# SvenGronauer/distributedTensorFlow

Hardware: AMD Instinct MI355X
Metric: images/sec (whole node) ResNet-50 synthetic ImageNet at 1/2/4/8 MI355X (higher is better)
Workload: dtype bf16; 1 GPU; model=resnet50, global_batch=1984, per_gpu_batch=1984, image_size=224, parallelism=dp1, impl=dtf, optimizer=momentum0.9+wd1e-4, lr 0.1*B/256 warmup500+cosine, backend=auto, native_ext=distributedtensorflow_amd/_lib/_dtf_hip.cpython-310-x86_64-linux-gnu.so

## Files before the change

csrc/kernels/gemm.hip:

```cpp
#include <algorithm>
#include <stdexcept>
#include <string>

#include "launch.h"

namespace {

constexpr int kGT = 512;
constexpr uint32_t kGOOB = 0xFFFFFFF0u;

struct GemmArgs {
  const bf16_t* A; const bf16_t* B; bf16_t* C;
  const float* bias;
  const bf16_t* Cin;
  int M, N, K, lda, ldb, ldc;
  int relu;
  float* stats;
  const bf16_t* acc_src;
  const uint8_t* acc_mask;
  int H, W, Cc, P, Q, sh, sw, ntaps;
  int tdh[9], tdw[9];
  int Ho, Wo, osh, osw, oh0, ow0;
  int nt;
  int dbg;
  const bf16_t* gelu_a;
  const float* gelu_b;
  float* colsum;
  bf16_t* gelu_out;
  int ncu;
  int group_m;
  int stagger_mode, stagger;
};

template <int BK>
DTF_DEV int gswz(int row, int ch) {
  constexpr int CPR = BK / 8, RPB = 16 / CPR;
  return ch ^ ((row / RPB) % CPR);
}

template <int BM, int BN, int BK, int NS, int NW = 8>
struct GCfg {
  static constexpr int NT = NW * 64;
  static constexpr int WN = NW == 8 ? BN / 64 : 2, WM = NW / WN;
  static constexpr int WTM = BM / WM, WTN = BN / WN;
  static constexpr int FM = WTM / 16, FN = WTN / 16;
  static constexpr int CPR = BK / 8;
  static constexpr int RPI = 64 / CPR;
  static constexpr int DA = BM / RPI / NW, DB = BN / RPI / NW;
  static constexpr int SA = BM * BK, STAGE = (BM + BN) * BK;
  static constexpr int LDC = BN + 8;
  static constexpr size_t EPI = (size_t)BM * LDC * 2 + (size_t)WM * 2 * BN * 4;
  static constexpr size_t LDS = (size_t)NS * STAGE * 2 > EPI ? (size_t)NS * STAGE * 2 : EPI;
};

template <int BM, int BN, int BK, int NS, int SCHED = 0, int NW = 8, int PP_PRIO = 1,
          int CONV = 0, int OCC = 1>
__global__ void __launch_bounds__(NW * 64, OCC == 2 ? NW * 2 / 4 : 1)
gemm_nt_kernel(const GemmArgs g) {
  using Cf = GCfg<BM, BN, BK, NS, NW>;
  extern __shared__ __attribute__((aligned(16))) bf16_t lds[];
  const int tid = threadIdx.x, lane = tid & 63;
  const int wave = __builtin_amdgcn_readfirstlane(tid >> 6);
  const int wm = wave / Cf::WN, wn = wave % Cf::WN;
  (void)kGT;

  const int tiles_n = (g.N + BN - 1) / BN;
  const int tiles_m = (g.M + BM - 1) / BM;
  const int bid = xcd_remap(blockIdx.x, tiles_n * tiles_m);
  int tm, tn;
  if (g.group_m > 0) {
    const int per = g.group_m * tiles_n, grp = bid / per, first = grp * g.group_m;
    const int gm = min(g.group_m, tiles_m - first), r = bid - grp * per;
    tm = first + r % gm;
    tn = r / gm;
  } else {
    tm = bid / tiles_n;
    tn = bid % tiles_n;
  }
  const int m0 = tm * BM, n0 = tn * BN;
  const int nk = (g.K + BK - 1) / BK;
  if constexpr (OCC == 2) {
    const int b = blockIdx.x;
    const bool late = b < 2 * g.ncu &&
        (g.stagger_mode == 1 ? b >= g.ncu
         : g.stagger_mode == 2 ? ((b >> 3) & 1) != 0
         : g.stagger_mode == 3 ? (b & 1) != 0 : false);
    if (late)
      for (int i = 0; i < g.stagger; ++i) __builtin_amdgcn_s_sleep(127);
  }

  const int rows_a = min(BM, g.M - m0), rows_b = min(BN, g.N - n0);
  const int PQc = CONV ? g.P * g.Q : 1;
  const int n_lo = CONV ? m0 / PQc : 0;
  const long img = CONV ? (long)g.H * g.W * g.Cc : 0;
  const i32x4_t ra =
      CONV ? rsrc_quad(g.A + n_lo * img,
                       (uint32_t)(((m0 + rows_a - 1) / PQc - n_lo + 1) * img * 2))
           : rsrc_quad(g.A + (long)m0 * g.lda, (uint32_t)((long)(rows_a - 1) * g.lda + g.K) * 2u);
  const i32x4_t rb = rsrc_quad(g.B + (long)n0 * g.ldb, (uint32_t)((long)(rows_b - 1) * g.ldb + g.K) * 2u);
  const uint32_t lds0 = lds_addr(lds);

  const int lrow = lane / Cf::CPR, slot = lane % Cf::CPR;
  uint32_t a_off[Cf::DA], b_off[Cf::DB];
  int a_ch[Cf::DA], b_ch[Cf::DB];
// ... 762 lines not shown
        float v[4];
        bf16_t h[4];
#pragma unroll
        for (int r = 0; r < 4; ++r) {
          v[r] = acc[i][j][r] + b4[r];
          if (g.relu) v[r] = fmaxf(v[r], 0.f);
          h[r] = f2bf(v[r]);
          if (do_stats && ok) {
            const float qv = bf2f(h[r]);
            s1[r] += qv;
            s2[r] += qv * qv;
          }
        }
        const long eoff = rowoff[i] + ncol;
        if (ok && (g.Cin || g.acc_mask)) {
          const bf16_t* src = g.Cin ? g.Cin + cbase + eoff : g.acc_src + cbase + eoff;
          const uint2 sv = *reinterpret_cast<const uint2*>(src);
          const uint32_t bits = g.Cin ? 0xFu
                                      : (g.acc_mask[(cbase + eoff) >> 3] >> ((cbase + eoff) & 7)) & 0xFu;
          const float s[4] = {__builtin_bit_cast(float, sv.x << 16),
                              __builtin_bit_cast(float, sv.x & 0xffff0000u),
                              __builtin_bit_cast(float, sv.y << 16),
                              __builtin_bit_cast(float, sv.y & 0xffff0000u)};
#pragma unroll
          for (int r = 0; r < 4; ++r) h[r] = f2bf(bf2f(h[r]) + ((bits >> r) & 1u ? s[r] : 0.f));
        }
        typedef uint32_t u32x2_t __attribute__((ext_vector_type(2)));
        const u32x2_t w = {(uint32_t)h[0] | ((uint32_t)h[1] << 16),
                           (uint32_t)h[2] | ((uint32_t)h[3] << 16)};
        const int so = ok ? (int)(eoff * 2) : (int)kGOOB;
        if (nt_store) __builtin_amdgcn_raw_buffer_store_b64(w, rc, so, 0, 2);
        else __builtin_amdgcn_raw_buffer_store_b64(w, rc, so, 0, 0);
      }
      if (do_stats) {
#pragma unroll
        for (int r = 0; r < 4; ++r) {
#pragma unroll
          for (int o = 1; o < 16; o <<= 1) {
            s1[r] += __shfl_xor(s1[r], o, 64);
            s2[r] += __shfl_xor(s2[r], o, 64);
          }
        }
        if (frow == 0) {
          const int col = wn * 64 + j * 16 + fq * 4;
#pragma unroll
          for (int r = 0; r < 4; ++r) {
            red[(wm * 2 + 0) * BN + col + r] = s1[r];
            red[(wm * 2 + 1) * BN + col + r] = s2[r];
          }
        }
      }
    }
    if (do_stats) {
      asm volatile("s_waitcnt lgkmcnt(0)" ::: "memory");
      raw_barrier();
      if (tid < BN && cur.n0 + tid < g.N) {
        float a = 0.f, b = 0.f;
#pragma unroll
        for (int k = 0; k < Cf::WM; ++k) { a += red[(k * 2 + 0) * BN + tid]; b += red[(k * 2 + 1) * BN + tid]; }
        const int tm = cur.m0 / BM;
        g.stats[((long)tm * 2 + 0) * g.N + cur.n0 + tid] = a;
        g.stats[((long)tm * 2 + 1) * g.N + cur.n0 + tid] = b;
      }
      asm volatile("s_waitcnt lgkmcnt(0)" ::: "memory");
      raw_barrier();
    }
    if (!nxt_valid) break;
#pragma unroll
    for (int i = 0; i < Cf::FM; ++i)
#pragma unroll
      for (int j = 0; j < Cf::FN; ++j) acc[i][j] = (f32x4_t){0.f, 0.f, 0.f, 0.f};
    gstep0 += nk;
    cur = tile_of(seq + 1);
    nxt_valid = tile_of(seq + 2).valid;
    ra = desc_a(cur);
    rb = desc_b(cur);
    cache();
    first = false;
    static_assert(NSTORE == 32, "the counted waits below assume 32 stores per lane per tile");
  }
  DTF_WAIT_VM(0);
}

template <int CONV, int EPI>
__global__ void __launch_bounds__(512, 1)
gemm_pp2_kernel(const GemmArgs g) {
  using Cf = GCfg<256, 256, 64, 2, 8>;
  constexpr int BM = 256, BN = 256, BK = 64;
  constexpr int NSTORE = Cf::FM * Cf::FN;
  extern __shared__ __attribute__((aligned(16))) bf16_t lds[];
  const int tid = threadIdx.x, lane = tid & 63;
  const int wave = __builtin_amdgcn_readfirstlane(tid >> 6);
  const int wm = wave / Cf::WN, wn = wave % Cf::WN;
  const int tiles_n = (g.N + BN - 1) / BN, tiles_m = (g.M + BM - 1) / BM;
  const int ntiles = tiles_n * tiles_m;
  const int nk = g.K / BK;
  const uint32_t lds0 = lds_addr(lds);
  const int lrow = lane / Cf::CPR, slot = lane % Cf::CPR;
  const int frow = lane & 15, fq = lane >> 4;
  const int PQc = CONV ? g.P * g.Q : 1;
  constexpr bool strided = CONV && (EPI & 4);
  const int cb = CONV ? g.Cc / BK : 1;

  auto prow = [&](int pc, int j) {
    const int r0 = pc == 0 ? j * 128 + 8 * wave
                 : pc == 3 ? 64 + j * 128 + 8 * wave
                           : (2 * j + (wave >> 2)) * 64 + (pc == 2 ? 32 : 0) + (wave & 3) * 8;
    return r0 + lrow;
  };
  const int pch = gswz<BK>(prow(0, 0), slot) * 8;
  constexpr bool ILV = true;
  auto plds = [&](int pc, int j) {
    const bool isA = pc == 0 || pc == 3;
    return (uint32_t)((isA ? 0 : Cf::SA) + (prow(pc, j) - lrow) * BK) * 2u;
  };
  const i32x4_t ra = rsrc_quad(g.A, (uint32_t)g.ncu);
  const i32x4_t rb = rsrc_quad(g.B, (uint32_t)g.group_m);

  auto tile_mn = [&](int seq, int& m0, int& n0) {
    const long phys = (long)blockIdx.x + (long)seq * gridDim.x;
    if (phys >= ntiles) { m0 = -1; n0 = 0; return false; }
    const int bid = xcd_remap((int)phys, ntiles);
    m0 = (bid / tiles_n) * BM;
    n0 = (bid % tiles_n) * BN;
    return true;
  };
  auto tile_offsets = [&](bool valid, int m0, int n0, uint32_t (&o)[4][2], int (&pk)[2][2]) {
#pragma unroll
    for (int pc = 0; pc < 4; ++pc)
#pragma unroll
      for (int j = 0; j < 2; ++j) {
        const bool isA = pc == 0 || pc == 3;
        const int row = prow(pc, j);
        if (isA) {
          const int m = m0 + row;
          const bool ok = valid && m < g.M;
          if constexpr (CONV) {
            const int mm = ok ? m : 0;
            const int q = mm % g.Q, t = mm / g.Q;
            const int p = t % g.P, n = t / g.P;
            pk[pc == 3][j] = (n << 20) | ((ok ? p * g.sh : 1023) << 10) | (q * g.sw);
            o[pc][j] = 0x80000000u;
          } else {
            o[pc][j] = ok ? (uint32_t)(m * g.lda + pch) * 2u : 0x80000000u;
          }
        } else {
          const int rho = row & 63;
          const int nl = ILV ? (row & ~63) + 4 * (rho & 15) + 2 * (rho >> 5) + ((rho >> 4) & 1)
                             : row;
          const int n = n0 + nl;
          const bool ok = valid && n < g.N;
          o[pc][j] = ok ? (uint32_t)(n * g.ldb + pch) * 2u : 0x80000000u;
        }
      }
  };

  int seq = 0, cm0, cn0, xm0, xn0;
  if (!tile_mn(0, cm0, cn0)) return;
  bool nxt_valid = tile_mn(1, xm0, xn0);
  uint32_t ocur[4][2], onxt[4][2];
  int pcur[2][2], pnxt[2][2];
  tile_offsets(true, cm0, cn0, ocur, pcur);
  tile_offsets(nxt_valid, xm0, xn0, onxt, pnxt);
  int gstep0 = 0;

  auto issue_piece = [&](int kt, int pc) {
    const bool nx = kt >= nk;
    const int kk = nx ? kt - nk : kt;
    const uint32_t base = lds0 + (uint32_t)(((gstep0 + kt) & 1) * Cf::STAGE) * 2u;
    const bool isA = pc == 0 || pc == 3;
    if constexpr (CONV) {
      if (isA) {
        const int tap = kk / cb, c0 = (kk % cb) * BK;
        const int dh = g.tdh[tap], dw = g.tdw[tap];
        const bool live = !nx || nxt_valid;
#pragma unroll
        for (int j = 0; j < 2; ++j) {
          const int v = nx ? pnxt[pc == 3][j] : pcur[pc == 3][j];
          const int h = ((v >> 10) & 1023) + dh, w = (v & 1023) + dw;
          const bool ok = live && (unsigned)h < (unsigned)g.H && (unsigned)w < (unsigned)g.W;
          dma16(ra, base + plds(pc, j),
                ok ? (uint32_t)((((v >> 20) * g.H + h) * g.W + w) * g.Cc + c0 + pch) * 2u : kGOOB);
        }
        return;
      }
    }
#pragma unroll
    for (int j = 0; j < 2; ++j) {
      const uint32_t o = nx ? onxt[pc][j] : ocur[pc][j];
      dma16(isA ? ra : rb, base + plds(pc, j), o + (uint32_t)(kk * BK) * 2u);
    }
  };

  f32x4_t acc[Cf::FM][Cf::FN];
#pragma unroll
  for (int i = 0; i < Cf::FM; ++i)
#pragma unroll
    for (int j = 0; j < Cf::FN; ++j) acc[i][j] = (f32x4_t){0.f, 0.f, 0.f, 0.f};

  bf16x8_t fA[8], fBl[4], fBr[4];
  auto rdA = [&](const bf16_t* sa, int half) {
#pragma unroll
    for (int ks = 0; ks < 2; ++ks)
#pragma unroll
      for (int i = 0; i < 4; ++i) {
        const int r = wm * 128 + half * 64 + i * 16 + frow, ch = ks * 4 + fq;
        fA[ks * 4 + i] = *reinterpret_cast<const bf16x8_t*>(sa + r * BK + gswz<BK>(r, ch) * 8);
      }
  };
  auto rdB = [&](bf16x8_t* fb, const bf16_t* sa, int half) {
    const bf16_t* sb = sa + Cf::SA;
#pragma unroll
    for (int ks = 0; ks < 2; ++ks)
#pragma unroll
      for (int j = 0; j < 2; ++j) {
        const int r = wn * 64 + half * 32 + j * 16 + frow, ch = ks * 4 + fq;
        fb[ks * 2 + j] = *reinterpret_cast<const bf16x8_t*>(sb + r * BK + gswz<BK>(r, ch) * 8);
      }
  };
  auto sync = [&]() {
    __builtin_amdgcn_sched_barrier(0);
    raw_barrier();
    __builtin_amdgcn_sched_barrier(0);
  };
  auto mfma_phase = [&](const bf16x8_t* fb, int ah, int bh) {
    sync();
    asm volatile("s_waitcnt lgkmcnt(0)" ::: "memory");
    __builtin_amdgcn_s_setprio(1);
#pragma unroll
    for (int ks = 0; ks < 2; ++ks)
#pragma unroll
      for (int i = 0; i < 4; ++i)
#pragma unroll
        for (int j = 0; j < 2; ++j)
          acc[ah * 4 + i][bh * 2 + j] = ILV
              ? __builtin_amdgcn_mfma_f32_16x16x32_bf16(fA[ks * 4 + i], fb[ks * 2 + j],
                                                        acc[ah * 4 + i][bh * 2 + j], 0, 0, 0)
              : __builtin_amdgcn_mfma_f32_16x16x32_bf16(fb[ks * 2 + j], fA[ks * 4 + i],
                                                        acc[ah * 4 + i][bh * 2 + j], 0, 0, 0);
    __builtin_amdgcn_s_setprio(0);
    sync();
  };

  float* red = reinterpret_cast<float*>(lds + 2 * Cf::STAGE);
  constexpr bool gelu_fwd = (EPI & 8) != 0, gelu_bwd = (EPI & 16) != 0;
  static_assert(!((gelu_fwd || gelu_bwd) && (EPI & 7)), "GELU epilogues are plain dense ones");
  auto wait_after_stores = [&]() {
    if constexpr (gelu_fwd) DTF_WAIT_VM(63);
    else DTF_WAIT_VM(40);
  };
  constexpr bool do_stats = (EPI & 1) != 0;
  constexpr bool has_acc = (EPI & 2) != 0;
  constexpr bool relu = (EPI & 32) != 0;
  static_assert(!relu || !(EPI & (1 | 4 | 8 | 16)), "ReLU: the plain / accumulate dense epilogues");

  issue_piece(0, 0); issue_piece(0, 1); issue_piece(0, 2); issue_piece(0, 3);
  issue_piece(1, 0); issue_piece(1, 1);
  DTF_WAIT_VM(8);
  bool first = true;
  for (;; ++seq) {
    sync();
    if (wm == 1) sync();
    for (int kt = 0; kt < nk; ++kt) {
      const bf16_t* cur_lds = lds + ((gstep0 + kt) & 1) * Cf::STAGE;
      rdB(fBl, cur_lds, 0);
      __builtin_amdgcn_sched_barrier(0);
      rdA(cur_lds, 0);
      issue_piece(kt + 1, 2);
      if (!first && kt == 0) wait_after_stores(); else DTF_WAIT_VM(8);
      mfma_phase(fBl, 0, 0);
      rdB(fBr, cur_lds, 1);
      issue_piece(kt + 1, 3);
      if (!first && kt == 0) wait_after_stores(); else DTF_WAIT_VM(8);
      mfma_phase(fBr, 0, 1);
      rdA(cur_lds, 1);
      issue_piece(kt + 2, 0);
      DTF_WAIT_VM(8);
      mfma_phase(fBr, 1, 1);
      issue_piece(kt + 2, 1);
      DTF_WAIT_VM(8);
      mfma_phase(fBl, 1, 0);
    }
    if (wm == 0) sync();

    const int n_lo = CONV ? cm0 / PQc : 0;
    const int rows_a = min(BM, g.M - cm0);
    long cbase;
    uint32_t cbytes;
    if (strided) {
      const int n_hi = (cm0 + rows_a - 1) / PQc;
      cbase = (long)n_lo * g.Ho * g.Wo * g.ldc;
      cbytes = (uint32_t)((long)(n_hi - n_lo + 1) * g.Ho * g.Wo * g.ldc * 2);
    } else {
      cbase = (long)cm0 * g.ldc;
      cbytes = (uint32_t)(((long)(rows_a - 1) * g.ldc + g.N) * 2);
    }
    const __amdgpu_buffer_rsrc_t rc =
        __builtin_amdgcn_make_buffer_rsrc(g.C + cbase, 0, (int)cbytes, 0x00020000);
    const bool nt_store = g.nt != 0;
    typedef uint32_t u32x2_t __attribute__((ext_vector_type(2)));
    if constexpr (ILV) {
      const int ncol = cn0 + wn * 64 + 4 * frow;
      const bool col_ok = ncol < g.N;
      float b4[4] = {0.f, 0.f, 0.f, 0.f};
      if (!do_stats && g.bias && col_ok) {
        const float4 bv = *reinterpret_cast<const float4*>(g.bias + ncol);
        b4[0] = bv.x; b4[1] = bv.y; b4[2] = bv.z; b4[3] = bv.w;
      }
      float s1[4] = {0.f, 0.f, 0.f, 0.f}, s2[4] = {0.f, 0.f, 0.f, 0.f};
      float gb4[4] = {0.f, 0.f, 0.f, 0.f};
      if (gelu_bwd && g.gelu_b && col_ok) {
        const float4 bv = *reinterpret_cast<const float4*>(g.gelu_b + ncol);
        gb4[0] = bv.x; gb4[1] = bv.y; gb4[2] = bv.z; gb4[3] = bv.w;
      }
      const __amdgpu_buffer_rsrc_t rg = __builtin_amdgcn_make_buffer_rsrc(
          gelu_fwd ? (void*)(g.gelu_out + cbase) : gelu_bwd ? (void*)(g.gelu_a + cbase) : (void*)g.C,
          0, (gelu_fwd || gelu_bwd) ? (int)cbytes : 0, 0x00020000);
      int vo = col_ok ? ((wm * 128 + fq * 4) * g.ldc + ncol) * 2 : (int)0x80000000u;
      const int ldc2 = g.ldc * 2;
      int* rtab = reinterpret_cast<int*>(red + Cf::WM * 2 * BN) + wave * 128;
      const int colb = col_ok ? ncol * 2 : (int)0x80000000u;
      if constexpr (strided) {
#pragma unroll
        for (int t = 0; t < 2; ++t) {
          const int m = cm0 + wm * 128 + lane + 64 * t;
          int o = (int)0x80000000u;
          if (m < g.M) {
            const int q = m % g.Q, tt = m / g.Q;
            const int p = tt % g.P, n = tt / g.P;
            o = ((((n - n_lo) * g.Ho + p * g.osh + g.oh0) * g.Wo + q * g.osw + g.ow0) * g.ldc) * 2;
          }
          rtab[lane + 64 * t] = o;
        }
        asm volatile("s_waitcnt lgkmcnt(0)" ::: "memory");
      }
      auto rows4 = [&](int i) -> i32x4_t {
        return *reinterpret_cast<const i32x4_t*>(rtab + 16 * i + 4 * fq);
      };
      const __amdgpu_buffer_rsrc_t rcin = __builtin_amdgcn_make_buffer_rsrc(
          has_acc ? const_cast<bf16_t*>(g.Cin ? g.Cin + cbase : g.acc_src + cbase) : g.C, 0,
          has_acc ? (int)cbytes : 0, 0x00020000);
      const __amdgpu_buffer_rsrc_t rmask = __builtin_amdgcn_make_buffer_rsrc(
          (has_acc && !g.Cin) ? const_cast<uint8_t*>(g.acc_mask + (cbase >> 3)) : (uint8_t*)g.C,
          0, (has_acc && !g.Cin) ? (int)(cbytes / 16) : 0, 0x00020000);
      constexpr bool has_ld = has_acc || gelu_bwd;
      typedef uint32_t u32x2l_t __attribute__((ext_vector_type(2)));
      const __amdgpu_buffer_rsrc_t rld = gelu_bwd ? rg : rcin;
      const bool masked = has_acc && !g.Cin;
      const int mshift = ncol & 7;
      u32x2l_t pa[4], pn[4];
      uint32_t pm[4], pmn[4];
      auto load_rows = [&](int vrow, int fi, u32x2l_t (&d)[4], uint32_t (&m)[4]) {
        i32x4_t t4 = {0, 0, 0, 0};
        if constexpr (strided) t4 = rows4(fi);
#pragma unroll
        for (int r = 0; r < 4; ++r) {
          const int o = strided ? (col_ok ? t4[r] + colb : (int)0x80000000u) : vrow + r * ldc2;
          d[r] = __builtin_bit_cast(u32x2l_t, __builtin_amdgcn_raw_buffer_load_b64(rld, o, 0, 0));
          m[r] = masked ? (uint32_t)__builtin_amdgcn_raw_buffer_load_b8(rmask, o >> 4, 0, 0) : 0u;
        }
      };
      if constexpr (has_ld) load_rows(vo, 0, pa, pm);
#pragma unroll
      for (int i = 0; i < Cf::FM; ++i) {
        if constexpr (has_ld) {
          if (i + 1 < Cf::FM) load_rows(vo + 16 * ldc2, i + 1, pn, pmn);
        }
        i32x4_t t4 = {0, 0, 0, 0};
        if constexpr (strided) t4 = rows4(i);
#pragma unroll
        for (int r = 0; r < 4; ++r) {
          const int vr = strided ? (col_ok ? t4[r] + colb : (int)0x80000000u) : vo + r * ldc2;
          bf16_t h[4];
#pragma unroll
          for (int jj = 0; jj < 4; ++jj) {
            float v = acc[i][jj][r] + b4[jj];
            if (relu) v = fmaxf(v, 0.f);
            h[jj] = f2bf(v);
            if (do_stats) {
              const float qv = bf2f(h[jj]);
              s1[jj] += qv;
              s2[jj] += qv * qv;
            }
          }
          if constexpr (has_acc) {
            const u32x2l_t sv = pa[r];
            const uint32_t bits = masked ? (pm[r] >> mshift) & 0xFu : 0xFu;
            const float sf[4] = {__builtin_bit_cast(float, sv.x << 16),
                                 __builtin_bit_cast(float, sv.x & 0xffff0000u),
                                 __builtin_bit_cast(float, sv.y << 16),
                                 __builtin_bit_cast(float, sv.y & 0xffff0000u)};
#pragma unroll
            for (int jj = 0; jj < 4; ++jj)
              h[jj] = f2bf(bf2f(h[jj]) + ((bits >> jj) & 1u ? sf[jj] : 0.f));
          }
          if constexpr (gelu_bwd) {
            const u32x2l_t av = pa[r];
            const float af[4] = {__builtin_bit_cast(float, av.x << 16),
                                 __builtin_bit_cast(float, av.x & 0xffff0000u),
                                 __builtin_bit_cast(float, av.y << 16),
                                 __builtin_bit_cast(float, av.y & 0xffff0000u)};
#pragma unroll
            for (int jj = 0; jj < 4; ++jj) {
              const float d = bf2f(h[jj]) * gelu_grad(af[jj] + gb4[jj]);
              s1[jj] += d;
              h[jj] = f2bf(d);
            }
          }
          const u32x2_t w = {(uint32_t)h[0] | ((uint32_t)h[1] << 16),
                             (uint32_t)h[2] | ((uint32_t)h[3] << 16)};
          if (nt_store) __builtin_amdgcn_raw_buffer_store_b64(w, rc, vr, 0, 2);
          else __builtin_amdgcn_raw_buffer_store_b64(w, rc, vr, 0, 0);
          if constexpr (gelu_fwd) {
            bf16_t q[4];
#pragma unroll
            for (int jj = 0; jj < 4; ++jj) q[jj] = f2bf(gelu_f(bf2f(h[jj])));
            const u32x2_t wq = {(uint32_t)q[0] | ((uint32_t)q[1] << 16),
                                (uint32_t)q[2] | ((uint32_t)q[3] << 16)};
            if (nt_store) __builtin_amdgcn_raw_buffer_store_b64(wq, rg, vr, 0, 2);
            else __builtin_amdgcn_raw_buffer_store_b64(wq, rg, vr, 0, 0);
          }
        }
        asm volatile("v_add_u32 %0, %0, %1" : "+v"(vo) : "s"(16 * ldc2));
        if constexpr (has_ld) {
#pragma unroll
          for (int r = 0; r < 4; ++r) { pa[r] = pn[r]; pm[r] = pmn[r]; }
        }
        __builtin_amdgcn_sched_barrier(0);
      }
      if constexpr (gelu_bwd) {
#pragma unroll
// ... 62 lines not shown
      float s1[4] = {0.f, 0.f, 0.f, 0.f}, s2[4] = {0.f, 0.f, 0.f, 0.f};
#pragma unroll
      for (int i = 0; i < Cf::FM; ++i) {
        const bool ok = col_ok && rowoff[i] >= 0;
        float v[4];
        bf16_t h[4];
#pragma unroll
        for (int r = 0; r < 4; ++r) {
          v[r] = acc[i][j][r] + b4[r];
          if (relu) v[r] = fmaxf(v[r], 0.f);
          h[r] = f2bf(v[r]);
          if (do_stats && ok) {
            const float qv = bf2f(h[r]);
            s1[r] += qv;
            s2[r] += qv * qv;
          }
        }
        const int eoff = rowoff[i] + ncol;
        if (has_acc && ok) {
          const bf16_t* src = g.Cin ? g.Cin + cbase + eoff : g.acc_src + cbase + eoff;
          const uint2 sv = *reinterpret_cast<const uint2*>(src);
          const uint32_t bits = g.Cin ? 0xFu
                                      : (g.acc_mask[(cbase + eoff) >> 3] >> ((cbase + eoff) & 7)) & 0xFu;
          const float sf[4] = {__builtin_bit_cast(float, sv.x << 16),
                               __builtin_bit_cast(float, sv.x & 0xffff0000u),
                               __builtin_bit_cast(float, sv.y << 16),
                               __builtin_bit_cast(float, sv.y & 0xffff0000u)};
#pragma unroll
          for (int r = 0; r < 4; ++r) h[r] = f2bf(bf2f(h[r]) + ((bits >> r) & 1u ? sf[r] : 0.f));
        }
        const u32x2_t w = {(uint32_t)h[0] | ((uint32_t)h[1] << 16),
                           (uint32_t)h[2] | ((uint32_t)h[3] << 16)};
        const int so = ok ? eoff * 2 : (int)kGOOB;
        if (nt_store) __builtin_amdgcn_raw_buffer_store_b64(w, rc, so, 0, 2);
        else __builtin_amdgcn_raw_buffer_store_b64(w, rc, so, 0, 0);
      }
      if (do_stats) {
#pragma unroll
        for (int r = 0; r < 4; ++r) {
#pragma unroll
          for (int o = 1; o < 16; o <<= 1) {
            s1[r] += __shfl_xor(s1[r], o, 64);
            s2[r] += __shfl_xor(s2[r], o, 64);
          }
        }
        if (frow == 0) {
          const int col = wn * 64 + j * 16 + fq * 4;
#pragma unroll
          for (int r = 0; r < 4; ++r) {
            red[(wm * 2 + 0) * BN + col + r] = s1[r];
            red[(wm * 2 + 1) * BN + col + r] = s2[r];
          }
        }
      }
    }
    }
    if (do_stats) {
      asm volatile("s_waitcnt lgkmcnt(0)" ::: "memory");
      raw_barrier();
      if (tid < BN && cn0 + tid < g.N) {
        float a = 0.f, b = 0.f;
#pragma unroll
        for (int k = 0; k < Cf::WM; ++k) { a += red[(k * 2 + 0) * BN + tid]; b += red[(k * 2 + 1) * BN + tid]; }
        const int tm = cm0 / BM;
        g.stats[((long)tm * 2 + 0) * g.N + cn0 + tid] = a;
        g.stats[((long)tm * 2 + 1) * g.N + cn0 + tid] = b;
      }
      asm volatile("s_waitcnt lgkmcnt(0)" ::: "memory");
      raw_barrier();
    }
    if (!nxt_valid) break;
#pragma unroll
    for (int i = 0; i < Cf::FM; ++i)
#pragma unroll
      for (int j = 0; j < Cf::FN; ++j) acc[i][j] = (f32x4_t){0.f, 0.f, 0.f, 0.f};
    gstep0 += nk;
    cm0 = xm0;
    cn0 = xn0;
#pragma unroll
    for (int pc = 0; pc < 4; ++pc)
#pragma unroll
      for (int j = 0; j < 2; ++j) ocur[pc][j] = onxt[pc][j];
#pragma unroll
    for (int a = 0; a < 2; ++a)
#pragma unroll
      for (int j = 0; j < 2; ++j) pcur[a][j] = pnxt[a][j];
    nxt_valid = tile_mn(seq + 2, xm0, xn0);
    tile_offsets(nxt_valid, xm0, xn0, onxt, pnxt);
    first = false;
    static_assert(NSTORE == 32, "the counted waits assume 32 stores per lane per tile");
  }
  DTF_WAIT_VM(0);
}

template <int CONV, int EPI>
void launch_gemm_pp2_t(const GemmArgs& g0, long a_bytes, long b_bytes, hipStream_t st) {
  using Cf = GCfg<256, 256, 64, 2, 8>;
  constexpr size_t LDS = (size_t)2 * Cf::STAGE * 2 + (size_t)Cf::WM * 2 * 256 * 4 +
                         ((EPI & 4) ? (size_t)8 * 128 * 4 : 0);
  static bool attr = false;
  static int ncu = 0;
  if (!attr) {
    HIP_CHECK(hipFuncSetAttribute((const void*)gemm_pp2_kernel<CONV, EPI>,
                                  hipFuncAttributeMaxDynamicSharedMemorySize, (int)LDS));
    hipFuncAttributes fa{};
    HIP_CHECK(hipFuncGetAttributes(&fa, (const void*)gemm_pp2_kernel<CONV, EPI>));
    if (fa.localSizeBytes > 0)
      throw std::runtime_error("gemm_pp2_kernel was compiled with register spills (scratch " +
                               std::to_string(fa.localSizeBytes) + " B/lane)");
    int dev = 0;
    HIP_CHECK(hipGetDevice(&dev));
    HIP_CHECK(hipDeviceGetAttribute(&ncu, hipDeviceAttributeMultiprocessorCount, dev));
    attr = true;
  }
  if (a_bytes <= 0 || a_bytes >= 0x7FFFFF00L || b_bytes <= 0 || b_bytes >= 0x7FFFFF00L ||
      g0.K % 64 || g0.K < 128)
    throw std::runtime_error("gemm_pp2: operands below 2^31 bytes, K % 64 == 0, K >= 128");
  GemmArgs g = g0;
  g.ncu = (int)a_bytes;
  g.group_m = (int)b_bytes;
  const long tiles = (long)((g.M + 255) / 256) * ((g.N + 255) / 256);
  long grid = tiles < ncu ? tiles : (ncu / 8) * 8;
  if (grid < 1) grid = 1;
  hipLaunchKernelGGL((gemm_pp2_kernel<CONV, EPI>), dim3((unsigned)grid), dim3(Cf::NT), LDS,
                     st, g);
}

template <int CONV>
void launch_gemm_pp2(const GemmArgs& g, long a_bytes, long b_bytes, hipStream_t st) {
  const bool stats = g.stats != nullptr, acc = g.Cin || g.acc_mask;
  const bool strided = CONV && (g.osh != 1 || g.osw != 1);
  if (g.relu && (CONV || stats || strided || g.gelu_out || g.gelu_a))
    throw std::runtime_error("gemm_pp2: ReLU only on the plain / accumulate dense epilogues");
  if constexpr (!CONV) {
    if (g.gelu_out) { launch_gemm_pp2_t<0, 8>(g, a_bytes, b_bytes, st); return; }
    if (g.gelu_a) { launch_gemm_pp2_t<0, 16>(g, a_bytes, b_bytes, st); return; }
    if (g.relu) {
      if (acc) launch_gemm_pp2_t<0, 34>(g, a_bytes, b_bytes, st);
      else launch_gemm_pp2_t<0, 32>(g, a_bytes, b_bytes, st);
      return;
    }
  }
  if (strided) {
    if (acc) launch_gemm_pp2_t<CONV, 6>(g, a_bytes, b_bytes, st);
    else launch_gemm_pp2_t<CONV, 4>(g, a_bytes, b_bytes, st);
  } else if (stats) {
    launch_gemm_pp2_t<CONV, 1>(g, a_bytes, b_bytes, st);
  } else if (acc) {
    launch_gemm_pp2_t<CONV, 2>(g, a_bytes, b_bytes, st);
  } else {
    launch_gemm_pp2_t<CONV, 0>(g, a_bytes, b_bytes, st);
  }
}

template <int CONV>
void launch_gemm_pp(const GemmArgs& g, hipStream_t st) {
  using Cf = GCfg<256, 256, 64, 2, 8>;
  constexpr size_t LDS = (size_t)2 * Cf::STAGE * 2 + (size_t)Cf::WM * 2 * 256 * 4;
  static bool attr = false;
  static int ncu = 0;
  if (!attr) {
    HIP_CHECK(hipFuncSetAttribute((const void*)gemm_pp_kernel<CONV>,
                                  hipFuncAttributeMaxDynamicSharedMemorySize, (int)LDS));
    hipFuncAttributes fa{};
    HIP_CHECK(hipFuncGetAttributes(&fa, (const void*)gemm_pp_kernel<CONV>));
    if (fa.localSizeBytes > 0)
      throw std::runtime_error("gemm_pp_kernel was compiled with register spills (scratch " +
                               std::to_string(fa.localSizeBytes) + " B/lane)");
    int dev = 0;
    HIP_CHECK(hipGetDevice(&dev));
    HIP_CHECK(hipDeviceGetAttribute(&ncu, hipDeviceAttributeMultiprocessorCount, dev));
    attr = true;
  }
  const long tiles = (long)((g.M + 255) / 256) * ((g.N + 255) / 256);
  long grid = tiles < ncu ? tiles : (ncu / 8) * 8;
  if (grid < 1) grid = 1;
  hipLaunchKernelGGL((gemm_pp_kernel<CONV>), dim3((unsigned)grid), dim3(Cf::NT), LDS, st, g);
}

int g_gemm_pp = 0;
int g_gemm_pp2 = 3;
int g_gemm_pp2_strided = 1;
int g_gemm_stream = 1;

int g_gemm_variant = -1;
int g_gemm_nt = 1;
int g_gemm_dbg = 0;

int g_gemm_stagger_mode = 1, g_gemm_stagger = -1;
int g_gemm_group = 0;

template <int BM, int BN, int BK, int NS, int SCHED = 0, int NW = 8, int PP_PRIO = 1,
          int CONV = 0, int OCC = 1>
void launch_gemm(const GemmArgs& g0, hipStream_t st) {
  using Cf = GCfg<BM, BN, BK, NS, NW>;
  static bool attr = false;
  static int ncu = 0;
  if (!attr) {
    HIP_CHECK(hipFuncSetAttribute(
        (const void*)gemm_nt_kernel<BM, BN, BK, NS, SCHED, NW, PP_PRIO, CONV, OCC>,
        hipFuncAttributeMaxDynamicSharedMemorySize, (int)Cf::LDS));
    int dev = 0;
    HIP_CHECK(hipGetDevice(&dev));
    HIP_CHECK(hipDeviceGetAttribute(&ncu, hipDeviceAttributeMultiprocessorCount, dev));
    attr = true;
  }
  static_assert(OCC == 1 || 2 * Cf::LDS <= 160 * 1024, "OCC 2: two blocks' LDS per CU");
  GemmArgs g = g0;
  if (!CONV) g.group_m = g_gemm_group;
  const long tiles = (long)((g.M + BM - 1) / BM) * ((g.N + BN - 1) / BN);
  if (OCC == 2) {
    g.ncu = ncu;
    g.stagger_mode = tiles > ncu ? g_gemm_stagger_mode : 0;
    g.stagger = g_gemm_stagger >= 0 ? g_gemm_stagger : ((g.K + BK - 1) / BK + 7) / 8;
  }
  hipLaunchKernelGGL((gemm_nt_kernel<BM, BN, BK, NS, SCHED, NW, PP_PRIO, CONV, OCC>),
                     dim3((unsigned)tiles), dim3(Cf::NT), Cf::LDS, st, g);
}

}

void dtf_gemm_set_variant(int v) { g_gemm_variant = v; }
void dtf_gemm_set_stream(int v) { g_gemm_stream = v; }
void dtf_gemm_set_pp(int v) { g_gemm_pp = v; }
void dtf_gemm_set_pp2(int v) { g_gemm_pp2 = v; }
void dtf_gemm_set_pp2_strided(int v) { g_gemm_pp2_strided = v; }
int dtf_gemm_get_pp2() { return g_gemm_pp2; }
void dtf_gemm_set_nt(int v) { g_gemm_nt = v; }
void dtf_gemm_set_dbg(int v) { g_gemm_dbg = v; }
void dtf_gemm_set_stagger(int mode, int iters) { g_gemm_stagger_mode = mode; g_gemm_stagger = iters; }
void dtf_gemm_set_group(int gm) { g_gemm_group = gm < 0 ? 0 : gm; }

int dtf_gemm_conv_part_images(int N, int H, int W, int C, int P, int Q) {
  const long img = (long)H * W * C * 2;
  if ((long)N * img < 0x7FFFFF00L) return 0;
  long a = (long)P * Q, b = 256;
  while (b) { const long t = a % b; a = b; b = t; }
  const long unit = 256 / a;
  const long per = (0x7FFFFF00L / img) / unit * unit;
  return per >= 1 && per < N && N < 2048 && H < 1000 && W < 1000 ? (int)per : -1;
}

void dtf_gemm_conv(const bf16_t* X, const bf16_t* Wt, bf16_t* Y, int N, int H, int W, int C,
                   int P, int Q, int sh, int sw, int Kout, int ntaps, const int* dh, const int* dw,
                   int Ho, int Wo, int osh, int osw, int oh0, int ow0,
                   float* stats, const bf16_t* Cin, const bf16_t* acc_src,
                   const uint8_t* acc_mask, hipStream_t st) {
  if (C % 64 || Kout % 8 || ntaps < 1 || ntaps > 9 || H >= 16384 || W >= 32768)
    throw std::runtime_error("gemm_conv: C % 64, Kout % 8, 1..9 taps, H < 2^14, W < 2^15");
  const long M = (long)N * P * Q;
  if (M >= (1L << 31) || 2.0 * H * W * C * (256.0 / (P * Q) + 2) >= 2147483647.0)
    throw std::runtime_error("gemm_conv: tile span too large for 32-bit buffer offsets");
  GemmArgs g{};
  g.A = X; g.B = Wt; g.C = Y; g.Cin = Cin; g.stats = stats; g.acc_src = acc_src;
  g.acc_mask = acc_mask;
  g.M = (int)M; g.N = Kout; g.K = ntaps * C; g.lda = C; g.ldb = ntaps * C; g.ldc = Kout;
  g.H = H; g.W = W; g.Cc = C; g.P = P; g.Q = Q; g.sh = sh; g.sw = sw; g.ntaps = ntaps;
  for (int t = 0; t < ntaps; ++t) { g.tdh[t] = dh[t]; g.tdw[t] = dw[t]; }
  g.Ho = Ho; g.Wo = Wo; g.osh = osh; g.osw = osw; g.oh0 = oh0; g.ow0 = ow0;
  g.nt = g_gemm_nt;
  if ((osh != 1 || osw != 1) && (stats || acc_mask))
    throw std::runtime_error("gemm_conv: strided outputs take no BN statistics / masked acc");
  if ((long)256 * g.ldb * 2 + 2L * g.K >= (1L << 31))
    throw std::runtime_error("gemm_conv: filter too large");
  const bool pp_span = !(osh != 1 || osw != 1) ||
      (256.0 / (P * Q) + 2) * Ho * Wo * (double)Kout * 2 < 2147483647.0;
  const long x_bytes = (long)N * H * W * C * 2, w_bytes = (long)Kout * g.ldb * 2;
  const int part_n = dtf_gemm_conv_part_images(N, H, W, C, P, Q);
  if (part_n > 0 && part_n < N && Kout > 128 && osh == 1 && osw == 1 && !Cin && !acc_src &&
      (g_gemm_pp2 & 2)) {
    const long pq = (long)P * Q;
    for (int n0 = 0; n0 < N; n0 += part_n) {
      const int cnt = std::min(part_n, N - n0);
      dtf_gemm_conv(X + (long)n0 * H * W * C, Wt, Y + (long)n0 * pq * Kout, cnt, H, W, C, P, Q, sh,
                    sw, Kout, ntaps, dh, dw, Ho, Wo, osh, osw, oh0, ow0,
                    stats ? stats + (long)n0 * pq / 256 * 2 * Kout : nullptr, nullptr, nullptr,
                    nullptr, st);
    }
    return;
  }
  if (Kout <= 128) launch_gemm<256, 128, 64, 3, 3, 8, 1, 1>(g, st);
  else if ((g_gemm_pp2 & 2) && (g_gemm_pp2_strided || (osh == 1 && osw == 1)) && g.K >= 128 &&
           x_bytes < 0x7FFFFF00L && w_bytes < 0x7FFFFF00L && N < 2048 && H < 1000 && W < 1000 &&
           pp_span)
    launch_gemm_pp2<1>(g, x_bytes, w_bytes, st);
  else if ((g_gemm_pp & 2) && (g.K + 63) / 64 >= 2 && pp_span) launch_gemm_pp<1>(g, st);
  else launch_gemm<256, 256, 64, 2, 2, 8, 1, 1>(g, st);
}

void dtf_gemm_nt_gelu_bwd(const bf16_t* A, const bf16_t* B, bf16_t* C, int M, int N, int K,
                          int lda, int ldb, const bf16_t* gelu_a, const float* gelu_b,
                          float* colsum, hipStream_t st) {
  if (M <= 0 || N <= 0 || K <= 0) return;
  if (K % 8 || N % 8 || lda % 8 || ldb % 8 || lda < K || ldb < K || !gelu_a || !colsum)
    throw std::runtime_error("gemm_nt_gelu_bwd: K, N, leading dims % 8; gelu_a and colsum needed");
  if ((long)256 * lda * 2 + 2L * K >= (1L << 31) || (long)256 * ldb * 2 + 2L * K >= (1L << 31))
    throw std::runtime_error("gemm_nt_gelu_bwd: leading dimension too large");
  GemmArgs g{};
  g.A = A; g.B = B; g.C = C; g.M = M; g.N = N; g.K = K; g.lda = lda; g.ldb = ldb; g.ldc = N;
  g.gelu_a = gelu_a; g.gelu_b = gelu_b; g.colsum = colsum;
  g.nt = g_gemm_nt;
  if (N <= 128) launch_gemm<256, 128, 64, 3>(g, st);
  else if ((g_gemm_pp2 & 1) && dtf_gemm_pp2_ok(M, N, K, lda, ldb) && N % 4 == 0)
    launch_gemm_pp2<0>(g, (long)(M - 1) * lda * 2 + 2L * K, (long)(N - 1) * ldb * 2 + 2L * K, st);
  else launch_gemm<256, 256, 64, 2, 2>(g, st);
}

void dtf_gemm_nt_bias_gelu(const bf16_t* A, const bf16_t* B, bf16_t* Z, bf16_t* H, int M, int N,
                           int K, int lda, int ldb, const float* bias, hipStream_t st) {
  if (M <= 0 || N <= 0 || K <= 0) return;
  if (K % 8 || N % 8 || lda % 8 || ldb % 8 || lda < K || ldb < K || !bias || !H)
    throw std::runtime_error("gemm_nt_bias_gelu: K, N, leading dims % 8; bias and H needed");
  if ((long)256 * lda * 2 + 2L * K >= (1L << 31) || (long)256 * ldb * 2 + 2L * K >= (1L << 31))
    throw std::runtime_error("gemm_nt_bias_gelu: leading dimension too large");
  GemmArgs g{};
  g.A = A; g.B = B; g.C = Z; g.M = M; g.N = N; g.K = K; g.lda = lda; g.ldb = ldb; g.ldc = N;
  g.bias = bias; g.gelu_out = H;
  g.nt = g_gemm_nt;
  if (N <= 128) launch_gemm<256, 128, 64, 3>(g, st);
  else if ((g_gemm_pp2 & 1) && dtf_gemm_pp2_ok(M, N, K, lda, ldb) && N % 4 == 0)
    launch_gemm_pp2<0>(g, (long)(M - 1) * lda * 2 + 2L * K, (long)(N - 1) * ldb * 2 + 2L * K, st);
  else launch_gemm<256, 256, 64, 2, 2>(g, st);
}

bool dtf_gemm_pp2_ok(int M, int N, int K, int lda, int ldb) {
  return K % 64 == 0 && K >= 128 && (long)(M - 1) * lda * 2 + 2L * K < 0x7FFFFF00L &&
         (long)(N - 1) * ldb * 2 + 2L * K < 0x7FFFFF00L;
}

int dtf_gemm_tile_rows(int M) { return (M + 255) / 256; }

void dtf_gemm_nt(const bf16_t* A, const bf16_t* B, bf16_t* C, int M, int N, int K, int lda,
                 int ldb, int ldc, const float* bias, const bf16_t* Cin, int relu, float* stats,
                 hipStream_t st, const bf16_t* acc_src, const uint8_t* acc_mask) {
  if (M <= 0 || N <= 0 || K <= 0) return;
  if (K % 8 || N % 8 || lda % 8 || ldb % 8 || ldc % 8 || lda < K || ldb < K || ldc < N)
    throw std::runtime_error("gemm_nt: K, N and the leading dimensions must be multiples of 8");
  if ((long)256 * lda * 2 + 2L * K >= (1L << 31) || (long)256 * ldb * 2 + 2L * K >= (1L << 31))
    throw std::runtime_error("gemm_nt: leading dimension too large");
  if (stats && (bias || relu || Cin))
    throw std::runtime_error("gemm_nt: BN statistics epilogue excludes bias / ReLU / accumulate");
  if (acc_mask && (!acc_src || Cin || ldc != N))
    throw std::runtime_error("gemm_nt: masked accumulation needs acc_src and a dense C");
  const bool stream_ok = !bias && !relu && (stats ? 1 : 0) + (Cin ? 1 : 0) +
      (acc_mask ? 1 : 0) <= 1 && dtf_gemm_stream_ok(M, N, K, lda, ldb, ldc);
  if (g_gemm_variant == 13 || (g_gemm_variant < 0 && g_gemm_stream && stream_ok && N >= K)) {
    if (!stream_ok) throw std::runtime_error("gemm_nt: shape not supported by variant 13");
    dtf_gemm_stream(A, B, C, M, N, K, lda, ldb, ldc, Cin, stats, acc_src, acc_mask, g_gemm_nt, st);
    return;
  }
  GemmArgs g{A, B, C, bias, Cin, M, N, K, lda, ldb, ldc, relu, stats, acc_src, acc_mask};
  g.nt = g_gemm_nt;
  g.dbg = g_gemm_dbg;
  const int variant = g_gemm_variant >= 0 ? g_gemm_variant
                    : (N <= 128 ? 1
                       : (g_gemm_pp2 & 1) && dtf_gemm_pp2_ok(M, N, K, lda, ldb) &&
                                 !(stats && (bias || relu)) ? 15
                       : ((g_gemm_pp & 1) && (K + 63) / 64 >= 2 ? 11 : 8));
  if (variant == 11 && (K + 63) / 64 < 2)
    throw std::runtime_error("gemm_nt: the persistent kernel needs K > 64");
  if (variant == 15 && (!dtf_gemm_pp2_ok(M, N, K, lda, ldb) || (stats && (bias || relu))))
    throw std::runtime_error("gemm_nt: shape not supported by the persistent kernel (variant 15)");
  switch (variant) {
    case 11: launch_gemm_pp<0>(g, st); break;
    case 15:
      launch_gemm_pp2<0>(g, (long)(M - 1) * lda * 2 + 2L * K, (long)(N - 1) * ldb * 2 + 2L * K, st);
      break;
// ... 15 lines not shown
```

Baseline: 16870 images/sec.

## Precompute conv tap offsets and validity bitmasks in pp2 implicit-GEMM loader

The pp2 implicit-GEMM conv kernel no longer decodes packed (n,h,w) coordinates and does per-load divisions and bounds checks for each K step. Each row now gets a precomputed base byte offset and a 16-bit row/column validity mask. A running tap cursor supplies a per-tap byte offset and selector bit, so the address becomes base+koff and validity a mask test. This cuts integer ALU work and register pressure in the A-load path, at the cost of a host-side tap table, a tap-span restriction (offsets under 8) that can route other convs to slower kernels, and some restructuring of the accumulate epilogue rules for strided outputs.

```diff
diff --git a/csrc/kernels/gemm.hip b/csrc/kernels/gemm.hip
--- a/csrc/kernels/gemm.hip
+++ b/csrc/kernels/gemm.hip
@@ -20,6 +20,8 @@
   const uint8_t* acc_mask;
   int H, W, Cc, P, Q, sh, sw, ntaps;
   int tdh[9], tdw[9];
+  int tsel[9][2];
+  int dh0, dw0;
   int Ho, Wo, osh, osw, oh0, ow0;
   int nt;
   int dbg;
@@ -948,7 +950,7 @@
   DTF_WAIT_VM(0);
 }
 
-template <int CONV, int EPI>
+template <int CONV, int EPI, bool TAP0 = false>
 __global__ void __launch_bounds__(512, 1)
 gemm_pp2_kernel(const GemmArgs g) {
   using Cf = GCfg<256, 256, 64, 2, 8>;
@@ -966,7 +968,6 @@
   const int frow = lane & 15, fq = lane >> 4;
   const int PQc = CONV ? g.P * g.Q : 1;
   constexpr bool strided = CONV && (EPI & 4);
-  const int cb = CONV ? g.Cc / BK : 1;
 
   auto prow = [&](int pc, int j) {
     const int r0 = pc == 0 ? j * 128 + 8 * wave
@@ -991,7 +992,9 @@
     n0 = (bid % tiles_n) * BN;
     return true;
   };
-  auto tile_offsets = [&](bool valid, int m0, int n0, uint32_t (&o)[4][2], int (&pk)[2][2]) {
+  auto tile_offsets = [&](bool valid, int m0, int n0, uint32_t (&o)[4][2], uint32_t (&pb)[2][2],
+                          uint32_t (&pv)[2]) {
+    if constexpr (CONV) pv[0] = pv[1] = 0u;
 #pragma unroll
     for (int pc = 0; pc < 4; ++pc)
 #pragma unroll
@@ -1005,7 +1008,12 @@
             const int mm = ok ? m : 0;
             const int q = mm % g.Q, t = mm / g.Q;
             const int p = t % g.P, n = t / g.P;
-            pk[pc == 3][j] = (n << 20) | ((ok ? p * g.sh : 1023) << 10) | (q * g.sw);
+            const int h0 = p * g.sh, w0 = q * g.sw;
+            pb[pc == 3][j] = (uint32_t)((((n * g.H + h0) * g.W + w0) * g.Cc + pch) * 2);
+            const int hlo = min(max(-(h0 + g.dh0), 0), 8), hhi = min(max(g.H - (h0 + g.dh0), hlo), 8);
+            const int wlo = min(max(-(w0 + g.dw0), 0), 8), whi = min(max(g.W - (w0 + g.dw0), wlo), 8);
+            const uint32_t bits = ((1u << hhi) - (1u << hlo)) | ((1u << whi) - (1u << wlo)) << 8;
+            pv[pc == 3] |= (ok ? bits : 0u) << (16 * j);
             o[pc][j] = 0x80000000u;
           } else {
             o[pc][j] = ok ? (uint32_t)(m * g.lda + pch) * 2u : 0x80000000u;
@@ -1025,28 +1033,35 @@
   if (!tile_mn(0, cm0, cn0)) return;
   bool nxt_valid = tile_mn(1, xm0, xn0);
   uint32_t ocur[4][2], onxt[4][2];
-  int pcur[2][2], pnxt[2][2];
-  tile_offsets(true, cm0, cn0, ocur, pcur);
-  tile_offsets(nxt_valid, xm0, xn0, onxt, pnxt);
+  uint32_t pbcur[2][2], pbnxt[2][2], pvcur[2], pvnxt[2];
+  tile_offsets(true, cm0, cn0, ocur, pbcur, pvcur);
+  tile_offsets(nxt_valid, xm0, xn0, onxt, pbnxt, pvnxt);
   int gstep0 = 0;
 
-  auto issue_piece = [&](int kt, int pc) {
+  struct TapCur { int tap, cs; uint32_t koff, sel; };
+  const int cc2 = CONV ? g.Cc * 2 : 0;
+  auto cur_step = [&](TapCur& c) {
+    if constexpr (TAP0) return;
+    c.cs += BK * 2;
+    const bool wrap = c.cs == cc2;
+    c.cs = wrap ? 0 : c.cs;
+    c.tap += wrap ? 1 : 0;
+    c.tap = c.tap == g.ntaps ? 0 : c.tap;
+  };
+
+  auto issue_piece = [&](int kt, int pc, const TapCur& ac) {
     const bool nx = kt >= nk;
     const int kk = nx ? kt - nk : kt;
     const uint32_t base = lds0 + (uint32_t)(((gstep0 + kt) & 1) * Cf::STAGE) * 2u;
     const bool isA = pc == 0 || pc == 3;
     if constexpr (CONV) {
       if (isA) {
-        const int tap = kk / cb, c0 = (kk % cb) * BK;
-        const int dh = g.tdh[tap], dw = g.tdw[tap];
-        const bool live = !nx || nxt_valid;
+        const uint32_t v = nx ? pvnxt[pc == 3] : pvcur[pc == 3];
 #pragma unroll
         for (int j = 0; j < 2; ++j) {
-          const int v = nx ? pnxt[pc == 3][j] : pcur[pc == 3][j];
-          const int h = ((v >> 10) & 1023) + dh, w = (v & 1023) + dw;
-          const bool ok = live && (unsigned)h < (unsigned)g.H && (unsigned)w < (unsigned)g.W;
-          dma16(ra, base + plds(pc, j),
-                ok ? (uint32_t)((((v >> 20) * g.H + h) * g.W + w) * g.Cc + c0 + pch) * 2u : kGOOB);
+          const uint32_t b = nx ? pbnxt[pc == 3][j] : pbcur[pc == 3][j];
+          const uint32_t s = ac.sel << (16 * j);
+          dma16(ra, base + plds(pc, j), (v & s) == s ? b + ac.koff : kGOOB);
         }
         return;
       }
@@ -1120,8 +1135,19 @@
   constexpr bool relu = (EPI & 32) != 0;
   static_assert(!relu || !(EPI & (1 | 4 | 8 | 16)), "ReLU: the plain / accumulate dense epilogues");
 
-  issue_piece(0, 0); issue_piece(0, 1); issue_piece(0, 2); issue_piece(0, 3);
-  issue_piece(1, 0); issue_piece(1, 1);
+  TapCur c1{0, 0, 0u, 0u}, c2{0, 0, 0u, 0u};
+  if constexpr (CONV) {
+    c1.koff = (uint32_t)g.tsel[0][0];
+    c1.sel = (uint32_t)g.tsel[0][1];
+    issue_piece(0, 0, c1); issue_piece(0, 1, c1); issue_piece(0, 2, c1); issue_piece(0, 3, c1);
+    cur_step(c1);
+    c1.koff = (uint32_t)(g.tsel[c1.tap][0] + c1.cs);
+    c1.sel = (uint32_t)g.tsel[c1.tap][1];
+    c2 = c1;
+  } else {
+    issue_piece(0, 0, c1); issue_piece(0, 1, c1); issue_piece(0, 2, c1); issue_piece(0, 3, c1);
+  }
+  issue_piece(1, 0, c1); issue_piece(1, 1, c1);
   DTF_WAIT_VM(8);
   bool first = true;
   for (;; ++seq) {
@@ -1129,23 +1155,35 @@
     if (wm == 1) sync();
     for (int kt = 0; kt < nk; ++kt) {
       const bf16_t* cur_lds = lds + ((gstep0 + kt) & 1) * Cf::STAGE;
+      int toff2 = 0, tsel2 = 0;
+      if constexpr (CONV) {
+        cur_step(c2);
+        toff2 = g.tsel[c2.tap][0];
+        tsel2 = g.tsel[c2.tap][1];
+      }
       rdB(fBl, cur_lds, 0);
       __builtin_amdgcn_sched_barrier(0);
       rdA(cur_lds, 0);
-      issue_piece(kt + 1, 2);
+      issue_piece(kt + 1, 2, c1);
       if (!first && kt == 0) wait_after_stores(); else DTF_WAIT_VM(8);
       mfma_phase(fBl, 0, 0);
       rdB(fBr, cur_lds, 1);
-      issue_piece(kt + 1, 3);
+      issue_piece(kt + 1, 3, c1);
       if (!first && kt == 0) wait_after_stores(); else DTF_WAIT_VM(8);
       mfma_phase(fBr, 0, 1);
+      if constexpr (CONV) {
+        c2.koff = (uint32_t)(toff2 + c2.cs);
+        c2.sel = (uint32_t)tsel2;
+        __builtin_amdgcn_sched_barrier(0);
+      }
       rdA(cur_lds, 1);
-      issue_piece(kt + 2, 0);
+      issue_piece(kt + 2, 0, c2);
       DTF_WAIT_VM(8);
       mfma_phase(fBr, 1, 1);
-      issue_piece(kt + 2, 1);
+      issue_piece(kt + 2, 1, c2);
       DTF_WAIT_VM(8);
       mfma_phase(fBl, 1, 0);
+      c1 = c2;
     }
     if (wm == 0) sync();
 
@@ -1155,8 +1193,10 @@
     uint32_t cbytes;
     if (strided) {
       const int n_hi = (cm0 + rows_a - 1) / PQc;
-      cbase = (long)n_lo * g.Ho * g.Wo * g.ldc;
-      cbytes = (uint32_t)((long)(n_hi - n_lo + 1) * g.Ho * g.Wo * g.ldc * 2);
+      int ho = g.Ho;
+      asm volatile("" : "+s"(ho));
+      cbase = (long)n_lo * ho * g.Wo * g.ldc;
+      cbytes = (uint32_t)((long)(n_hi - n_lo + 1) * ho * g.Wo * g.ldc * 2);
     } else {
       cbase = (long)cm0 * g.ldc;
       cbytes = (uint32_t)(((long)(rows_a - 1) * g.ldc + g.N) * 2);
@@ -1203,16 +1243,16 @@
       auto rows4 = [&](int i) -> i32x4_t {
         return *reinterpret_cast<const i32x4_t*>(rtab + 16 * i + 4 * fq);
       };
+      const bool masked = has_acc && !strided && !g.Cin;
       const __amdgpu_buffer_rsrc_t rcin = __builtin_amdgcn_make_buffer_rsrc(
-          has_acc ? const_cast<bf16_t*>(g.Cin ? g.Cin + cbase : g.acc_src + cbase) : g.C, 0,
+          has_acc ? const_cast<bf16_t*>(masked ? g.acc_src + cbase : g.Cin + cbase) : g.C, 0,
           has_acc ? (int)cbytes : 0, 0x00020000);
       const __amdgpu_buffer_rsrc_t rmask = __builtin_amdgcn_make_buffer_rsrc(
-          (has_acc && !g.Cin) ? const_cast<uint8_t*>(g.acc_mask + (cbase >> 3)) : (uint8_t*)g.C,
-          0, (has_acc && !g.Cin) ? (int)(cbytes / 16) : 0, 0x00020000);
+          masked ? const_cast<uint8_t*>(g.acc_mask + (cbase >> 3)) : (uint8_t*)g.C,
+          0, masked ? (int)(cbytes / 16) : 0, 0x00020000);
       constexpr bool has_ld = has_acc || gelu_bwd;
       typedef uint32_t u32x2l_t __attribute__((ext_vector_type(2)));
       const __amdgpu_buffer_rsrc_t rld = gelu_bwd ? rg : rcin;
-      const bool masked = has_acc && !g.Cin;
       const int mshift = ncol & 7;
       u32x2l_t pa[4], pn[4];
       uint32_t pm[4], pmn[4];
@@ -1441,18 +1481,20 @@
 #pragma unroll
       for (int j = 0; j < 2; ++j) ocur[pc][j] = onxt[pc][j];
 #pragma unroll
-    for (int a = 0; a < 2; ++a)
-#pragma unroll
-      for (int j = 0; j < 2; ++j) pcur[a][j] = pnxt[a][j];
+    for (int a = 0; a < 2; ++a) {
+      pvcur[a] = pvnxt[a];
+#pragma unroll
+      for (int j = 0; j < 2; ++j) pbcur[a][j] = pbnxt[a][j];
+    }
     nxt_valid = tile_mn(seq + 2, xm0, xn0);
-    tile_offsets(nxt_valid, xm0, xn0, onxt, pnxt);
+    tile_offsets(nxt_valid, xm0, xn0, onxt, pbnxt, pvnxt);
     first = false;
     static_assert(NSTORE == 32, "the counted waits assume 32 stores per lane per tile");
   }
   DTF_WAIT_VM(0);
 }
 
-template <int CONV, int EPI>
+template <int CONV, int EPI, bool TAP0 = false>
 void launch_gemm_pp2_t(const GemmArgs& g0, long a_bytes, long b_bytes, hipStream_t st) {
   using Cf = GCfg<256, 256, 64, 2, 8>;
   constexpr size_t LDS = (size_t)2 * Cf::STAGE * 2 + (size_t)Cf::WM * 2 * 256 * 4 +
@@ -1460,10 +1502,10 @@
   static bool attr = false;
   static int ncu = 0;
   if (!attr) {
-    HIP_CHECK(hipFuncSetAttribute((const void*)gemm_pp2_kernel<CONV, EPI>,
+    HIP_CHECK(hipFuncSetAttribute((const void*)gemm_pp2_kernel<CONV, EPI, TAP0>,
                                   hipFuncAttributeMaxDynamicSharedMemorySize, (int)LDS));
     hipFuncAttributes fa{};
-    HIP_CHECK(hipFuncGetAttributes(&fa, (const void*)gemm_pp2_kernel<CONV, EPI>));
+    HIP_CHECK(hipFuncGetAttributes(&fa, (const void*)gemm_pp2_kernel<CONV, EPI, TAP0>));
     if (fa.localSizeBytes > 0)
       throw std::runtime_error("gemm_pp2_kernel was compiled with register spills (scratch " +
                                std::to_string(fa.localSizeBytes) + " B/lane)");
@@ -1481,8 +1523,19 @@
   const long tiles = (long)((g.M + 255) / 256) * ((g.N + 255) / 256);
   long grid = tiles < ncu ? tiles : (ncu / 8) * 8;
   if (grid < 1) grid = 1;
-  hipLaunchKernelGGL((gemm_pp2_kernel<CONV, EPI>), dim3((unsigned)grid), dim3(Cf::NT), LDS,
+  hipLaunchKernelGGL((gemm_pp2_kernel<CONV, EPI, TAP0>), dim3((unsigned)grid), dim3(Cf::NT), LDS,
                      st, g);
+}
+
+template <int CONV, int EPI>
+void launch_gemm_pp2_e(const GemmArgs& g, long a_bytes, long b_bytes, hipStream_t st) {
+#ifdef DTF_PROBES
+  if (CONV && (g.dbg & 2)) {
+    launch_gemm_pp2_t<CONV, EPI, CONV != 0>(g, a_bytes, b_bytes, st);
+    return;
+  }
+#endif
+  launch_gemm_pp2_t<CONV, EPI>(g, a_bytes, b_bytes, st);
 }
 
 template <int CONV>
@@ -1491,6 +1544,8 @@
   const bool strided = CONV && (g.osh != 1 || g.osw != 1);
   if (g.relu && (CONV || stats || strided || g.gelu_out || g.gelu_a))
     throw std::runtime_error("gemm_pp2: ReLU only on the plain / accumulate dense epilogues");
+  if (strided && acc && !g.Cin)
+    throw std::runtime_error("gemm_pp2: strided output rows accumulate from Cin only");
   if constexpr (!CONV) {
     if (g.gelu_out) { launch_gemm_pp2_t<0, 8>(g, a_bytes, b_bytes, st); return; }
     if (g.gelu_a) { launch_gemm_pp2_t<0, 16>(g, a_bytes, b_bytes, st); return; }
@@ -1501,14 +1556,14 @@
     }
   }
   if (strided) {
-    if (acc) launch_gemm_pp2_t<CONV, 6>(g, a_bytes, b_bytes, st);
-    else launch_gemm_pp2_t<CONV, 4>(g, a_bytes, b_bytes, st);
+    if (acc) launch_gemm_pp2_e<CONV, 6>(g, a_bytes, b_bytes, st);
+    else launch_gemm_pp2_e<CONV, 4>(g, a_bytes, b_bytes, st);
   } else if (stats) {
-    launch_gemm_pp2_t<CONV, 1>(g, a_bytes, b_bytes, st);
+    launch_gemm_pp2_e<CONV, 1>(g, a_bytes, b_bytes, st);
   } else if (acc) {
-    launch_gemm_pp2_t<CONV, 2>(g, a_bytes, b_bytes, st);
+    launch_gemm_pp2_e<CONV, 2>(g, a_bytes, b_bytes, st);
   } else {
-    launch_gemm_pp2_t<CONV, 0>(g, a_bytes, b_bytes, st);
+    launch_gemm_pp2_e<CONV, 0>(g, a_bytes, b_bytes, st);
   }
 }
 
@@ -1615,9 +1670,18 @@
   g.acc_mask = acc_mask;
   g.M = (int)M; g.N = Kout; g.K = ntaps * C; g.lda = C; g.ldb = ntaps * C; g.ldc = Kout;
   g.H = H; g.W = W; g.Cc = C; g.P = P; g.Q = Q; g.sh = sh; g.sw = sw; g.ntaps = ntaps;
-  for (int t = 0; t < ntaps; ++t) { g.tdh[t] = dh[t]; g.tdw[t] = dw[t]; }
+  g.dh0 = *std::min_element(dh, dh + ntaps);
+  g.dw0 = *std::min_element(dw, dw + ntaps);
+  bool tap_span = true;
+  for (int t = 0; t < ntaps; ++t) {
+    g.tdh[t] = dh[t]; g.tdw[t] = dw[t];
+    tap_span = tap_span && dh[t] - g.dh0 < 8 && dw[t] - g.dw0 < 8;
+    g.tsel[t][0] = (int)(((long)dh[t] * W + dw[t]) * C * 2);
+    g.tsel[t][1] = tap_span ? 1 << (dh[t] - g.dh0) | 1 << (8 + dw[t] - g.dw0) : 0;
+  }
   g.Ho = Ho; g.Wo = Wo; g.osh = osh; g.osw = osw; g.oh0 = oh0; g.ow0 = ow0;
   g.nt = g_gemm_nt;
+  g.dbg = g_gemm_dbg & 2;
   if ((osh != 1 || osw != 1) && (stats || acc_mask))
     throw std::runtime_error("gemm_conv: strided outputs take no BN statistics / masked acc");
   if ((long)256 * g.ldb * 2 + 2L * g.K >= (1L << 31))
@@ -1641,7 +1705,7 @@
   if (Kout <= 128) launch_gemm<256, 128, 64, 3, 3, 8, 1, 1>(g, st);
   else if ((g_gemm_pp2 & 2) && (g_gemm_pp2_strided || (osh == 1 && osw == 1)) && g.K >= 128 &&
            x_bytes < 0x7FFFFF00L && w_bytes < 0x7FFFFF00L && N < 2048 && H < 1000 && W < 1000 &&
-           pp_span)
+           pp_span && tap_span)
     launch_gemm_pp2<1>(g, x_bytes, w_bytes, st);
   else if ((g_gemm_pp & 2) && (g.K + 63) / 64 >= 2 && pp_span) launch_gemm_pp<1>(g, st);
   else launch_gemm<256, 256, 64, 2, 2, 8, 1, 1>(g, st);
```

After: 17150 images/sec (median of 6 runs). +1.6%, better.
